# facebook/facebook360_dep

Measured on AMD Instinct MI355X. Metric: depth Mpix/s per GPU (full pyramid, 16-cam 2048^2 rig); % HBM-read roofline, higher is better.
Workload: dtype f32+f64; 1 GPU; BASELINE config 3: 16-camera 2048x2048 synthetic rig, 8-frame sequence, full 10-level pyramid per frame, per-level temporal filter (+-2 frames); the same sequence for every --gpus N (block partition, 8 frame(s) on this rank); rig=cfg2, cameras=16, frames=8, temporal_filter=True, halo_transport=local, parallelism=frames x1

## Files before the change

### facebook360_dep_amd/csrc/derp_capi.hip

```cpp
#include <hip/hip_runtime.h>

#include <algorithm>
#include <cfloat>
#include <cmath>
#include <cstdarg>
#include <cstdio>
#include <cstdlib>
#include <cstring>
#include <map>
#include <memory>
#include <string>
#include <vector>

#include <rocprim/device/device_radix_sort.hpp>

#include "../../include/derp_hip.h"
#include "derp_host.h"
#include "derp_kernels.h"
#include "derp_mesh.h"
#include "derp_points.h"
#include "derp_render.h"
#include "derp_geometric.h"
#include "derp_sweep.h"
#include "derp_align.h"
// ... 337 lines not shown
  return 0;
}

bool batch_needs_inverse_warps(const derp_ctx* c, int dst0, int nd) {
  std::vector<char> covered(c->S, 0);
  for (int d = dst0; d < dst0 + nd; ++d) {
    covered[c->dst2srcH[d]] = 1;
  }
  for (int s = 0; s < c->S; ++s) {
    if (!covered[s]) {
      return true;
    }
  }
  return false;
}

size_t table_bytes_per_dst(const derp_ctx* c, int W, int H, bool withInverse) {
  const size_t wp = (size_t)(W + 2 * kPadW) * (H + 2 * kPadW), cp = (size_t)(W + 2 * kPadC) * (H + 2 * kPadC);
  return (size_t)(c->S - 1) * (wp * sizeof(float2) + 2 * cp * sizeof(ushort4) + (withInverse ? (size_t)W * H * sizeof(float2) : 0) +
                               (DERP_RANDOM_TILED ? tiled_plane(W, H) * sizeof(ushort4) : 0));
}

int compute_fov_and_masks(derp_ctx* c, int level) {
  const int W = c->LW[level], H = c->LH[level];
  const size_t n = (size_t)W * H;
  {
    Span sp(c, ST_FOV, level);
    if (c->opt.rebuild_warp_tables || c->fovCachedLevel != level) {
      hipLaunchKernelGGL(k_fov_mask, grid2d(W, H, c->D, kBlk2d), kBlk2d, 0, c->stream, c->camsDst.as<Cam>(), W, H,
                         c->fovMask.as<uint8_t>());
      KCHECK(c);
      c->fovCachedLevel = level;
    }
    hipLaunchKernelGGL(k_and_masks, dim3(flat_grid(n), c->D), dim3(256), 0, c->stream, c->fovMask.as<uint8_t>(),
                       c->frame().fg[level].as<uint8_t>(), c->dst2src.as<int>(), 0, n, c->w.maskAnd.as<uint8_t>());
    KCHECK(c);
  }
  return 0;
}

int build_warp(derp_ctx* c, int dst0, int nd) {
  const int L = c->cur;
  Span sp(c, ST_PROJ_WARP, L);
  {
    const size_t n = (size_t)c->LW[L] * c->LH[L];
    ALLOC(c, c->rayDir, 3 * n * c->D * sizeof(double));
    ALLOC(c, c->behind, n * c->D * sizeof(unsigned));
  }
  LevelView V = make_view(c, ST_PROJ_WARP, dst0, nd);
  hipLaunchKernelGGL(k_proj_warp, grid2d(V.W + 2 * kPadW, V.H + 2 * kPadW, c->S, kBlk2d), kBlk2d, 0, c->stream, V,
                     c->projWarp.as<float2>());
  KCHECK(c);
  hipLaunchKernelGGL(k_pixel_rays, grid2d(V.W, V.H, nd, kBlk2d), kBlk2d, 0, c->stream, V, c->rayDir.as<double>(),
                     c->behind.as<unsigned>());
  KCHECK(c);
  c->w.colorTablesCleanLevel = -1;
  if (batch_needs_inverse_warps(c, dst0, nd)) {
    hipLaunchKernelGGL(k_proj_warp_inv, grid2d(V.W, V.H, nd, kBlk2d), kBlk2d, 0, c->stream, V, c->projWarpInv.as<float2>());
    KCHECK(c);
  }
  return 0;
}

int build_color_tables(derp_ctx* c, int dst0, int nd) {
  const int L = c->cur;
  LevelView V = make_view(c, ST_REPROJECT, dst0, nd);
  Span sp(c, ST_REPROJECT, L);
  const dim3 grid((V.W + kRbTile - 1) / kRbTile, (V.H + kRbTile - 1) / kRbTile, nd * (c->S - 1));
  ALLOC(c, c->w.tileSeen, (size_t)grid.x * grid.y * grid.z);
  const int skipBlank = c->w.colorTablesCleanLevel == L && nd == c->D && !c->noBlankSkip;
  const auto kernel = c->reprojectSerial ? k_reproject_bias : k_reproject_bias_front;
// ... 187 lines not shown
  return t * 4 * sizeof(float) + ((t + 3) & ~(size_t)3);
}

constexpr size_t kBilateralMaxLds = 64 * 1024 - 256;

bool bilateral_fast_tap_ok(float sigma, float w0, float w1, float w2) {
  const float denom = 2.0f * (sigma * sigma);
  return w1 == 1.0f && w2 == 1.0f && w0 >= 0.0f && std::isfinite(w0) && denom > 0.0f && std::isfinite(denom);
}

bool temporal_fast_tap_ok(float sigma, float w0, float w1, float w2) {
  const float sig2 = sigma * sigma;
  const auto weight_ok = [](float w) { return w >= 0.0f && std::isfinite(w); };
  return weight_ok(w0) && weight_ok(w1) && weight_ok(w2) && sig2 > 0.0f && std::isfinite(sig2);
}

void launch_joint_bilateral_u16_tiled(derp_ctx* c, dim3 grid, const float* image, const void* guide, const uint8_t* mask,
                                      int W, int H, int radius, float sigma, float w0, float w1, float w2, float* out,
                                      size_t planeStride, size_t guideStride, const int* guideIndex) {
  const bool fast = bilateral_fast_tap_ok(sigma, w0, w1, w2) && bilateral_lds_bytes(radius) + 256 <= kBilateralMaxLds;
  const auto kernel = fast ? k_joint_bilateral<true, true> : k_joint_bilateral<true, false>;
  hipLaunchKernelGGL(kernel, grid, dim3(256), bilateral_lds_bytes(radius), c->stream, image, guide, mask, W, H, radius, sigma,
                     w0, w1, w2, out, planeStride, guideStride, guideIndex);
}

int run_bilateral(derp_ctx* c) {
  const int L = c->cur;
  Span sp(c, ST_BILATERAL, L);
  c->randomRanThisLevel = false;
  const int W = c->LW[L], H = c->LH[L];
  const size_t n = (size_t)W * H;
  const int radius = bilateral_radius(L);
  launch_joint_bilateral_u16_tiled(c, dim3((W + 15) / 16, (H + 15) / 16, c->D), c->w.disparity.as<float>(),
                                   (const void*)c->frame().color[L].as<ushort4>(), c->w.maskAnd.as<uint8_t>(), W, H, radius,
                                   0.005f, 0.5f, 1.0f, 1.0f, c->w.tmpF.as<float>(), n, n, c->dst2src.as<int>());
  KCHECK(c);
  std::swap(c->w.disparity, c->w.tmpF);
  return 0;
}

int run_median(derp_ctx* c, bool fuseMaskFov, float* levelOut = nullptr) {
  const int L = c->cur;
  Span sp(c, ST_MEDIAN, L);
  c->randomRanThisLevel = false;
  const int W = c->LW[L], H = c->LH[L];
  const size_t n = (size_t)W * H;
  hipLaunchKernelGGL(k_masked_median, grid2d(W, H, c->D, kBlk2d), kBlk2d, 0, c->stream, c->w.disparity.as<float>(),
                     c->opt.use_foreground_masks ? c->frame().bg[L].as<float>() : (const float*)nullptr,
                     c->w.maskAnd.as<uint8_t>(), W, H, 1, levelOut ? levelOut : c->w.tmpF.as<float>(), n,
                     fuseMaskFov ? c->fovMask.as<uint8_t>() : (const uint8_t*)nullptr);
  KCHECK(c);
  if (!levelOut) {
    std::swap(c->w.disparity, c->w.tmpF);
  }
  return 0;
}

int run_mask_fov(derp_ctx* c, float* levelOut = nullptr) {
  const int L = c->cur;
  Span sp(c, ST_MASKFOV, L);
  const size_t n = npx(c, L) * c->D;
  hipLaunchKernelGGL(k_mask_fov, dim3(flat_grid(n)), dim3(256), 0, c->stream, c->w.disparity.as<float>(),
                     c->fovMask.as<uint8_t>(), levelOut ? levelOut : c->w.disparity.as<float>(), n);
  KCHECK(c);
  return 0;
}

int check_level(derp_ctx* c, int level) {
  if (!c || c->numLevels == 0) {
    return fail(c, "derp_set_pyramid has not been called");
  }
  if (level < 0 || level >= c->numLevels) {
    return fail(c, "level %d out of range [0, %d)", level, c->numLevels);
  }
  if (c->LW[level] <= 0 || c->LH[level] <= 0) {
    return fail(c, "level %d was declared absent in derp_set_pyramid", level);
  }
  return 0;
}

int level_begin(derp_ctx* c, int level, bool buildAllTables) {
  TRY(check_level(c, level));
// ... 253 lines not shown
  }
  if (n > kMaxTemporalFrames) {
    ALLOC(c, c->temporalCarry, (size_t)planes * W * H * sizeof(float2));
  }
  for (int t0 = 0; t0 < n; t0 += kMaxTemporalFrames) {
    TemporalFrames F;
    F.n = std::min(kMaxTemporalFrames, n - t0);
    for (int t = 0; t < F.n; ++t) {
      F.guides[t] = reinterpret_cast<const ushort4*>(guides[t0 + t]);
      F.images[t] = images[t0 + t];
      F.masks[t] = masks[t0 + t];
    }
    F.refGuide = reinterpret_cast<const ushort4*>(guides[centre]);
    F.refImage = images[centre];
    F.refMask = masks[centre];
    F.carry = n > kMaxTemporalFrames ? c->temporalCarry.as<float2>() : nullptr;
    F.first = t0 == 0;
    F.last = t0 + F.n >= n;
    const size_t lds = 2 * ((((size_t)(32 + 2 * radius) * (8 + 2 * radius) * 9) + 15) & ~(size_t)15);
    if (radius >= 0 && lds <= 48 * 1024 && !c->noTemporalTile) {
      const bool fast = temporal_fast_tap_ok(sigma, w0, w1, w2) && !c->temporalGeneric;
      const auto kernel = !fast ? k_temporal_tiled<-1, false> : radius == 1 ? k_temporal_tiled<1, true> : k_temporal_tiled<-1, true>;
      hipLaunchKernelGGL(kernel, grid2d(W, H, planes, kBlk2d), kBlk2d, lds, c->stream, F, W, H, sigma, radius, w0, w1, w2, out,
                         dst2src);
    } else {
      hipLaunchKernelGGL(k_temporal, grid2d(W, H, planes, kBlk2d), kBlk2d, 0, c->stream, F, W, H, sigma, radius, w0, w1, w2,
                         out, dst2src);
    }
    KCHECK(c);
  }
  return 0;
}

}

extern "C" {

void derp_options_default(derp_options* o) {
  o->min_depth_m = 0.5f;
  o->max_depth_m = 1e4f;
  o->var_noise_floor = 4e-5f;
  o->var_high_thresh = 1e-3f;
  o->random_proposals = 2;
  o->ping_pong_iterations = 1;
  o->mismatches_start_level = -1;
  o->do_bilateral_filter = 1;
  o->do_median_filter = 1;
  o->use_foreground_masks = 0;
  o->partial_coverage = 0;
  o->rebuild_warp_tables = 1;
}

int derp_create(derp_ctx** out, int device, const derp_camera_desc* src, int n_src, const derp_camera_desc* dst,
                int n_dst) {
  if (!out) {
    return 1;
  }
  *out = nullptr;
  std::unique_ptr<derp_ctx> owner(new derp_ctx);
  derp_ctx* c = owner.get();
  derp_options_default(&c->opt);
  if (n_src <= 0 || n_dst <= 0) {
    return create_fail("no source / destination cameras!");
  }
  hipDeviceProp_t prop;
  TRY(open_device(device, "the depth path", &prop));
  c->device = device;
  if (prop.maxSharedMemoryPerMultiProcessor > 0) {
    c->ldsPerCu = prop.maxSharedMemoryPerMultiProcessor;
  }
  if (const char* e = getenv("DERP_XCD_ROTATE")) {
    c->xcdRotate = atoi(e);
  }
  if (const char* e = getenv("DERP_XCD_BANDS")) {
    c->xcdBands = atoi(e);
  }
  if (const char* e = getenv("DERP_COST_TILES_PER_BLOCK")) {
    c->costTilesPerBlock = atoi(e);
  }
  c->noMemo = getenv("DERP_NO_MEMO") != nullptr;
  if (const char* e = getenv("DERP_BRUTE_RUN")) {
    c->bruteRun = atoi(e);
  }
  if (const char* e = getenv("DERP_PP_COMPACT")) {
    c->ppCompact = atoi(e) != 0;
  }
  if (const char* e = getenv("DERP_RANDOM_WAVES")) {
    c->randomWaves = atoi(e);
  }
  if (const char* e = getenv("DERP_PP_WAVES")) {
    c->ppWaves = atoi(e);
  }
  c->noTemporalTile = getenv("DERP_NO_TEMPORAL_TILE") != nullptr;
  c->noBlankSkip = getenv("DERP_NO_BLANK_SKIP") != nullptr;
  if (const char* e = getenv("DERP_TEMPORAL_GENERIC")) {
    c->temporalGeneric = atoi(e) != 0;
  }
  if (const char* e = getenv("DERP_REPROJECT_SERIAL")) {
    c->reprojectSerial = atoi(e) != 0;
  }
  c->S = n_src;
  c->D = n_dst;
  c->frames.resize(1);
  c->camsSrcH.resize(n_src);
  c->camsDstH.resize(n_dst);
  for (int i = 0; i < n_src; ++i) {
    if (const char* m = host_prepare_camera(src[i], c->camsSrcH[i])) {
      return create_fail(std::string("camera ") + src[i].id + ": " + m);
    }
  }
  c->dst2srcH.assign(n_dst, 0);
  c->descDstH.assign(dst, dst + n_dst);
  for (int i = 0; i < n_dst; ++i) {
    if (const char* m = host_prepare_camera(dst[i], c->camsDstH[i])) {
      return create_fail(std::string("camera ") + dst[i].id + ": " + m);
    }
    bool found = false;
    for (int s = 0; s < n_src; ++s) {
      if (strncmp(dst[i].id, src[s].id, sizeof dst[i].id) == 0) {
        c->dst2srcH[i] = s;
        found = true;
        break;
      }
    }
    if (!found) {
      return create_fail(std::string("destination camera ") + dst[i].id + " is not a source camera");
    }
    if (memcmp(&c->camsDstH[i], &c->camsSrcH[c->dst2srcH[i]], sizeof(Cam)) != 0) {
      return create_fail(std::string("destination camera ") + dst[i].id + " differs from the source camera of the same id "
                  "(destinations must be cameras of the source rig, as filterDestinations makes them)");
// ... 451 lines not shown
```

### facebook360_dep_amd/csrc/derp_ctx.h

```cpp
#pragma once

namespace {

enum Stage {
  ST_FOV = 0,
  ST_VARIANCE,
  ST_OWN_BIAS,
  ST_UPSAMPLE,
  ST_PROJ_WARP,
  ST_REPROJECT,
  ST_PROJ_BIAS,
  ST_BRUTE,
  ST_RANDOM,
  ST_PINGPONG,
  ST_MISMATCH,
  ST_BILATERAL,
  ST_MEDIAN,
  ST_MASKFOV,
  ST_TEMPORAL,
  ST_LANES,
  ST_GC_PREPARE,
  ST_GC_SWEEP,
  ST_GC_CLEAN,
  ST_SWEEP_OVERLAPS,
// ... 86 lines not shown
  DevBuf temporalCarry;
  DevBuf projWarp, projWarpInv;
  DevBuf rayDir, behind;
  int warpCachedLevel = -1;
  DevBuf fovMask;
  int fovCachedLevel = -1;
  bool randomRanThisLevel = false;
  bool tablesValid = false;
  std::map<std::pair<int, int>, LanczosTab> lanczos;
  std::map<std::pair<int, int>, AreaTabDev> areaTabs;
  DevBuf spiral;
  int spiralN = 0, spiralRadius = -1;
  std::vector<std::unique_ptr<WorkLane>> lanes;
  hipEvent_t laneReady = nullptr;
  int activeLane = -1;

  DevBuf counters;
  bool profiling = false;
  std::vector<TimedSpan> spans;
  double accMs[ST_COUNT][kMaxLevels] = {};
  int accLaunch[ST_COUNT][kMaxLevels] = {};
  int xcdRotate = 1;
  int xcdBands = 0, costTilesPerBlock = 0;
  DevBuf blockTrace[2][kMaxLevels];
  int blockTraceGrid[2][kMaxLevels][2] = {};
  bool noMemo = false;
  int bruteRun = 10;
  bool ppCompact = true;
  int randomWaves = 0, ppWaves = 0;
  size_t ldsPerCu = 160 * 1024;
  bool noTemporalTile = false;
  bool noBlankSkip = false;
  bool temporalGeneric = false, reprojectSerial = false;
  std::unique_ptr<SmrState> smr;
  std::unique_ptr<RephotoState> rephoto;
  std::unique_ptr<PointsState> points;
  std::unique_ptr<MeshState> mesh;
  std::unique_ptr<GcState> gc;
  std::unique_ptr<SweepState> sweep;
  std::unique_ptr<AlignState> align;
};

namespace {

int fail(derp_ctx* c, const char* fmt, ...) {
  va_list ap;
  va_start(ap, fmt);
  vfail(c ? &c->err : nullptr, fmt, ap);
  va_end(ap);
  return 1;
}

int use_device(derp_ctx* c) {
  if (!c) {
    return 1;
  }
  HIPCHK(c, hipSetDevice(c->device));
  return 0;
}

int check_camera(derp_ctx* c, int cam) {
  if (cam < 0 || cam >= c->D) {
    return fail(c, "bad camera index %d (the context has %d)", cam, c->D);
  }
  return 0;
}
// ... 3 lines not shown
```

### facebook360_dep_amd/csrc/derp_kernels.h

```cpp
#pragma once
#include <hip/hip_runtime.h>
#include <math.h>
#include <stdint.h>

#include <type_traits>

#include "derp_camera.h"
#include "gcc_algos.h"

namespace derp {

#ifndef DERP_COST_MIN_WAVES
#define DERP_COST_MIN_WAVES 4
#endif
#ifndef DERP_RANDOM_MIN_WAVES
#define DERP_RANDOM_MIN_WAVES 4
#endif
#ifndef DERP_RANDOM_TILED
#define DERP_RANDOM_TILED 0
#endif
#ifndef DERP_MIX_HOT_ONLY
#define DERP_MIX_HOT_ONLY 0
#endif
#ifndef DERP_PHASE_TIMERS
// ... 3013 lines not shown
        }
      } else {
        for (int u = -radius; u <= radius; ++u) {
          for (int v = -radius; v <= radius; ++v) {
            const int k = ((int)threadIdx.y + radius + v) * TW + (int)threadIdx.x + radius + u;
            if (!tm[k]) {
              continue;
            }
            temporal_tap<FAST>(ref, tg[k], centre, weight0, weight1, weight2, rcpSig2, expTab, weightedSumPix, sumWeight);
          }
        }
      }
    }
    if (t + 1 < F.n) {
      stash(t + 1);
    }
  }
  if (!inside) {
    return;
  }
  if (!active) {
    if (F.last) {
      out[pd + idx] = F.refImage[pd + idx];
    }
    return;
  }
  if (F.last) {
    out[pd + idx] = weightedSumPix / sumWeight;
  } else {
    F.carry[pd + idx] = make_float2(weightedSumPix, sumWeight);
  }
}

__global__ void k_rephoto_splat(const Cam* __restrict__ cams, int target, const float* __restrict__ disps, int W, int H,
                                unsigned long long* __restrict__ key) {
  const int x = blockIdx.x * blockDim.x + threadIdx.x, y = blockIdx.y * blockDim.y + threadIdx.y;
  const int j = blockIdx.z;
  if (x >= W || y >= H || j == target) {
    return;
  }
  const size_t n = (size_t)W * H, idx = (size_t)y * W + x;
  const float d = disps[(size_t)j * n + idx];
  if (!(d > 0) || isinf(d)) {
    return;
  }
  const Cam& cj = cams[j];
  const Cam& ct = cams[target];
  const D3 dir = rig_direction(cj, (x + 0.5) / (double)W, (y + 0.5) / (double)H, cj.principal[0], cj.principal[1],
                               cj.focal[0], cj.focal[1]);
  const double depth = (double)(1.0f / d);
  const D3 p = {cj.pos[0] + dir.x * depth, cj.pos[1] + dir.y * depth, cj.pos[2] + dir.z * depth};
  D2 pn;
  if (!sees(ct, p, ct.principal[0], ct.principal[1], ct.focal[0], ct.focal[1], 1.0, 1.0, pn)) {
    return;
  }
  const double px = pn.x * (double)W, py = pn.y * (double)H;
  const double dx = p.x - ct.pos[0], dy = p.y - ct.pos[1], dz = p.z - ct.pos[2];
  const float dist = (float)sqrt(sum3(dx * dx, dy * dy, dz * dz));
  const unsigned long long k =
      ((unsigned long long)__float_as_uint(dist) << 32) | ((unsigned long long)j << 24) | (unsigned long long)idx;
  const int x0 = (int)floor(px - 0.5), y0 = (int)floor(py - 0.5);
  for (int yy = y0; yy <= y0 + 1; ++yy) {
    for (int xx = x0; xx <= x0 + 1; ++xx) {
      if (xx >= 0 && yy >= 0 && xx < W && yy < H) {
        atomicMin(&key[(size_t)yy * W + xx], k);
      }
// ... 412 lines not shown
```

### facebook360_dep_amd/csrc/derp_sequence.h

```cpp
#pragma once
#include <dlfcn.h>
#include <rccl/rccl.h>

namespace {

void seq_window(int t, int first, int last, int radius, int* lo, int* hi) {
  *lo = std::max(first, t - radius);
  *hi = std::min(last, t + radius);
}

int seq_owner(int first, int last, int world, int policy, int frame) {
  const int F = last - first + 1, i = frame - first;
  if (i < 0 || i >= F || world < 1) {
    return -1;
  }
  if (policy == DERP_SEQ_CYCLIC) {
    return i % world;
  }
  const int q = F / world, r = F % world;
  const int big = r * (q + 1);
  return i < big ? i / (q + 1) : r + (q ? (i - big) / q : 0);
}

std::vector<derp_seq_transfer> seq_plan(int first, int last, int world, int radius, int policy) {
// ... 49 lines not shown
  auto sym = [&](const char* n) {
    void* p = dlsym(api.lib, n);
    if (!p && api.error.empty()) {
      api.error = std::string("librccl lacks ") + n;
    }
    return p;
  };
  api.GetUniqueId = reinterpret_cast<decltype(api.GetUniqueId)>(sym("ncclGetUniqueId"));
  api.CommInitRank = reinterpret_cast<decltype(api.CommInitRank)>(sym("ncclCommInitRank"));
  api.CommDestroy = reinterpret_cast<decltype(api.CommDestroy)>(sym("ncclCommDestroy"));
  api.GroupStart = reinterpret_cast<decltype(api.GroupStart)>(sym("ncclGroupStart"));
  api.GroupEnd = reinterpret_cast<decltype(api.GroupEnd)>(sym("ncclGroupEnd"));
  api.Send = reinterpret_cast<decltype(api.Send)>(sym("ncclSend"));
  api.Recv = reinterpret_cast<decltype(api.Recv)>(sym("ncclRecv"));
  api.GetErrorString = reinterpret_cast<decltype(api.GetErrorString)>(sym("ncclGetErrorString"));
  if (!api.error.empty()) {
    api.lib = nullptr;
  }
  return &api;
}

enum { SEQ_NONE = 0, SEQ_LOOPBACK = 1, SEQ_RCCL = 2, SEQ_EXTERNAL = 3 };

}

struct derp_seq {
  derp_ctx* c = nullptr;
  int first = 0, last = 0, rank = 0, world = 1;
  derp_seq_options opt;
  std::vector<int> owned, halo;
  std::vector<derp_seq_transfer> plan;
  std::vector<std::vector<DevBuf>> haloColor, haloFg, haloDisp;
  std::vector<DevBuf> filtered;
  DevBuf fov, winMask;
  int transport = SEQ_NONE;
  std::vector<derp_seq*> peers;
  ncclComm_t comm = nullptr;
  unsigned long long bytesSent = 0, bytesRecv = 0;
  std::vector<std::pair<hipEvent_t, hipEvent_t>> exchangeSpans;
  double exchangeMs = 0;
  hipStream_t xStream = nullptr;
  hipEvent_t computedEv = nullptr, exchangedEv = nullptr;
  bool exchangePending = false;
  std::vector<std::pair<hipEvent_t, hipEvent_t>> waitSpans;
  double exchangeExposedMs = 0;
  int levelReady = -1;
  int levelExchanged = -1;
  int computeLevel = -1, computedFrames = 0;
  std::vector<int> computedAt, filteredAt;
  std::vector<uint64_t> uploaded;
  std::vector<hipEvent_t> filteredEv;
  int fovLevel = -1;
  bool streaming = false;
  int nSlots = 0;
  struct HostIn {
    const uint16_t* color = nullptr;
    const uint8_t* fg = nullptr;
    const float* bg = nullptr;
  };
  std::vector<std::vector<HostIn>> hostIn;
  std::vector<std::vector<float*>> hostDisp;
  std::vector<char> hostHave;
  std::vector<float*> hostRaw;
  struct SlotTag {
    int k = -1, colorLevel = -1, rawLevel = -1;
  };
  std::vector<SlotTag> slotTag;
// ... 309 lines not shown
  if (hipSetDevice(c->device) != hipSuccess) {
    return fail(c, "hipSetDevice failed");
  }
  const int nOwned = (int)q->owned.size();
  q->streaming = q->opt.resident_frames > 0 && q->opt.resident_frames < nOwned;
  q->nSlots = q->streaming ? q->opt.resident_frames : std::max(1, nOwned);
  if (q->streaming && q->opt.do_temporal_filter && q->nSlots < 2 * q->opt.time_radius + 1) {
    return fail(c, "resident_frames %d is smaller than the temporal window (2 * time_radius + 1 = %d frames)",
                q->nSlots, 2 * q->opt.time_radius + 1);
  }
  TRY(derp_set_frame_slots(c, q->nSlots));
  const int nl = c->numLevels;
  for (auto* vv : {&q->haloColor, &q->haloFg, &q->haloDisp}) {
    vv->resize(q->halo.size());
    for (auto& v : *vv) {
      v.resize(nl);
    }
  }
  size_t nmax = 0;
  for (int l = 0; l < nl; ++l) {
    const size_t n = npx(c, l);
    nmax = std::max(nmax, n);
    if (n == 0) {
      continue;
    }
    for (size_t h = 0; h < q->halo.size(); ++h) {
      if (q->haloColor[h][l].ensure(n * c->S * sizeof(ushort4)) || q->haloDisp[h][l].ensure(n * c->D * sizeof(float)) ||
          (q->opt.use_foreground_masks && q->haloFg[h][l].ensure(n * c->S))) {
        return fail(c, "out of device memory allocating the temporal halo (frame %d, level %d)", q->halo[h], l);
      }
    }
  }
  q->filtered.resize(q->streaming ? 1 : q->owned.size());
  q->computedAt.assign(q->owned.size(), -1);
  q->filteredAt.assign(q->owned.size(), -1);
  if (hipStreamCreateWithFlags(&q->xStream, hipStreamNonBlocking) != hipSuccess ||
      hipEventCreateWithFlags(&q->computedEv, hipEventDisableTiming) != hipSuccess ||
      hipEventCreateWithFlags(&q->exchangedEv, hipEventDisableTiming) != hipSuccess) {
    return fail(c, "hipStreamCreate / hipEventCreate failed");
  }
  q->filteredEv.assign(q->streaming ? 0 : q->owned.size(), nullptr);
  for (auto& e : q->filteredEv) {
    if (hipEventCreateWithFlags(&e, hipEventDisableTiming) != hipSuccess) {
      return fail(c, "hipEventCreate failed");
    }
  }
  for (auto& b : q->filtered) {
    if (b.ensure(nmax * c->D * sizeof(float))) {
      return fail(c, "out of device memory allocating the filtered level");
    }
  }
  if (q->streaming) {
    q->slotTag.assign(q->nSlots, derp_seq::SlotTag());
    q->hostIn.assign(nOwned, std::vector<derp_seq::HostIn>(nl));
    q->hostDisp.assign(nOwned, std::vector<float*>(nl, nullptr));
    q->hostHave.assign((size_t)nOwned * nl, 0);
    q->hostRaw.assign(nOwned, nullptr);
    for (int k = 0; k < nOwned; ++k) {
      if (q->opt.do_temporal_filter && hipHostMalloc((void**)&q->hostRaw[k], nmax * c->D * sizeof(float), hipHostMallocDefault) != hipSuccess) {
        q->hostRaw[k] = nullptr;
        return fail(c, "out of page-locked host memory for the raw level of frame %d", q->owned[k]);
      }
      for (int l = 0; l < nl; ++l) {
        const size_t n = npx(c, l);
        if (n && hipHostMalloc((void**)&q->hostDisp[k][l], n * c->D * sizeof(float), hipHostMallocDefault) != hipSuccess) {
          q->hostDisp[k][l] = nullptr;
          return fail(c, "out of page-locked host memory for the results of frame %d", q->owned[k]);
        }
      }
    }
    for (const derp_seq_transfer& tr : q->plan) {
      if (tr.from_rank == rank && (q->edge.empty() || q->edge.back() != tr.frame)) {
        q->edge.push_back(tr.frame);
      }
    }
    for (auto* vv : {&q->edgeColor, &q->edgeFg}) {
      vv->resize(q->edge.size());
      for (auto& v : *vv) {
        v.resize(nl);
      }
    }
    q->edgeRaw.resize(q->edge.size());
    for (size_t e = 0; e < q->edge.size(); ++e) {
      if (q->edgeRaw[e].ensure(nmax * c->D * sizeof(float))) {
        return fail(c, "out of device memory allocating the edge frames");
      }
      for (int l = 0; l < nl; ++l) {
        const size_t n = npx(c, l);
        if (n && (q->edgeColor[e][l].ensure(n * c->S * sizeof(ushort4)) ||
                  (q->opt.use_foreground_masks && q->edgeFg[e][l].ensure(n * c->S)))) {
          return fail(c, "out of device memory allocating the edge frames");
        }
      }
    }
  }
  if (q->fov.ensure(nmax * c->D) ||
      (q->opt.use_foreground_masks && q->winMask.ensure((size_t)(2 * q->opt.time_radius + 1) * nmax * c->D))) {
    return fail(c, "out of device memory allocating the temporal masks");
  }
  *out = owner.release();
  return 0;
}

void derp_seq_destroy(derp_seq* q) {
  if (!q) {
    return;
  }
  if (q->c) {
    (void)hipSetDevice(q->c->device);
    (void)hipStreamSynchronize(q->c->stream);
  }
  seq_drain_spans(q);
  if (q->comm) {
    (void)rccl_api()->CommDestroy(q->comm);
  }
  for (auto& e : q->filteredEv) {
    if (e) {
      (void)hipEventDestroy(e);
    }
  }
  if (q->xStream) {
    (void)hipStreamSynchronize(q->xStream);
    (void)hipStreamDestroy(q->xStream);
  }
  for (hipEvent_t e : {q->computedEv, q->exchangedEv}) {
    if (e) {
      (void)hipEventDestroy(e);
    }
  }
  for (auto& v : q->hostDisp) {
// ... 629 lines not shown
  if (q->levelReady != level) {
    return fail(c, "derp_seq_level_exchange(%d): derp_seq_level_compute(%d) has not completed for every owned frame", level, level);
  }
  TRY(seq_exchange(q, level, 2));
  if (q->transport != SEQ_EXTERNAL) {
    q->levelExchanged = level;
  }
  if (q->streaming || getenv("DERP_SEQ_NO_OVERLAP")) {
    TRY(seq_join_exchange(q));
  }
  return 0;
}

int derp_seq_mark_exchanged(derp_seq* q, int level) {
  if (!q) {
    return 1;
  }
  q->levelExchanged = level;
  return 0;
}

namespace {
int seq_fov_masks(derp_seq* q, int level) {
  derp_ctx* c = q->c;
  if (q->fovLevel != level) {
    const int W = c->LW[level], H = c->LH[level];
    hipLaunchKernelGGL(k_fov_mask, grid2d(W, H, c->D, kBlk2d), kBlk2d, 0, c->stream, c->camsDst.as<Cam>(), W, H,
                       q->fov.as<uint8_t>());
    KCHECK(c);
    q->fovLevel = level;
  }
  return 0;
}
int seq_filter_frame(derp_seq* q, int level, int k) {
  derp_ctx* c = q->c;
  const int W = c->LW[level], H = c->LH[level];
  const size_t n = (size_t)W * H;
  const int radius = temporal_space_radius(q, level);
  const int t = q->owned[k];
  int lo, hi;
  seq_window(t, q->first, q->last, q->opt.time_radius, &lo, &hi);
  std::vector<const void*> wg(hi - lo + 1);
  std::vector<const float*> wi(hi - lo + 1);
  std::vector<const uint8_t*> wmk(hi - lo + 1);
  for (int u = lo; u <= hi; ++u) {
    void *pc, *pd, *pm;
    size_t b;
    TRY(seq_buffer(q, u, level, 0, &pc, &b));
    TRY(seq_buffer(q, u, level, 2, &pd, &b));
    if (q->opt.use_foreground_masks) {
      TRY(seq_buffer(q, u, level, 1, &pm, &b));
      uint8_t* wm = q->winMask.as<uint8_t>() + (size_t)(u - lo) * n * c->D;
      hipLaunchKernelGGL(k_and_masks, dim3(flat_grid(n), c->D), dim3(256), 0, c->stream, q->fov.as<uint8_t>(),
                         (const uint8_t*)pm, c->dst2src.as<int>(), 0, n, wm);
      KCHECK(c);
      pm = wm;
    } else {
      pm = q->fov.p;
    }
    wg[u - lo] = pc;
    wi[u - lo] = reinterpret_cast<const float*>(pd);
    wmk[u - lo] = reinterpret_cast<const uint8_t*>(pm);
  }
  TRY(temporal_launch(c, wg.data(), wi.data(), wmk.data(), hi - lo + 1, t - lo, W, H, c->D, q->opt.sigma, radius,
                      q->opt.weight_b, q->opt.weight_g, q->opt.weight_b, q->filtered[k].as<float>(), c->dst2src.as<int>()));
  q->filteredAt[k] = level;
  HIPCHK(c, hipEventRecord(q->filteredEv[k], c->stream));
  return 0;
}
}

int derp_seq_level_filter_frame(derp_seq* q, int level, int frame) {
  if (!q) {
    return 1;
  }
  derp_ctx* c = q->c;
  HIPCHK(c, hipSetDevice(c->device));
  TRY(check_level(c, level));
  const int k = owned_index(q, frame);
  if (k < 0) {
    return fail(c, "frame %d is not owned by rank %d", frame, q->rank);
  }
  if (!q->opt.do_temporal_filter || q->streaming) {
    return 2;
  }
  if (q->filteredAt[k] == level) {
    return 0;
  }
  int lo, hi;
  seq_window(frame, q->first, q->last, q->opt.time_radius, &lo, &hi);
  bool needsHalo = false;
  for (int u = lo; u <= hi; ++u) {
    const int ku = owned_index(q, u);
    if (ku >= 0 ? q->computedAt[ku] != level : q->levelExchanged != level) {
      return 2;
    }
    needsHalo |= ku < 0;
  }
  if (needsHalo) {
    TRY(seq_join_exchange(q));
  }
  Span sp(c, ST_TEMPORAL, level);
  TRY(seq_fov_masks(q, level));
  return seq_filter_frame(q, level, k);
}

int derp_seq_download_filtered(derp_seq* q, int frame, int level, int d, float* out) {
  if (!q) {
    return 1;
  }
  derp_ctx* c = q->c;
  TRY(check_level(c, level));
  const int k = owned_index(q, frame);
  if (k < 0 || d < -1 || d >= c->D || !out) {
    return fail(c, "bad frame / destination index / null output");
  }
  if (q->streaming || q->filteredAt[k] != level) {
    return fail(c, "frame %d has no filtered level %d in its scratch (derp_seq_level_filter_frame)", frame, level);
  }
  HIPCHK(c, hipSetDevice(c->device));
  const size_t n = npx(c, level);
  HIPCHK(c, hipStreamWaitEvent(c->copyStream, q->filteredEv[k], 0));
  HIPCHK(c, hipMemcpyAsync(out, q->filtered[k].as<float>() + (size_t)std::max(d, 0) * n, (d < 0 ? c->D : 1) * n * sizeof(float),
                           hipMemcpyDeviceToHost, c->copyStream));
  HIPCHK(c, hipStreamSynchronize(c->copyStream));
  return 0;
}

int derp_seq_level_filter(derp_seq* q, int level) {
  if (!q) {
    return 1;
  }
  derp_ctx* c = q->c;
  HIPCHK(c, hipSetDevice(c->device));
  TRY(check_level(c, level));
  if (!q->opt.do_temporal_filter) {
    return 0;
  }
  if (q->levelReady != level) {
    return fail(c, "derp_seq_level_filter(%d): derp_seq_level_compute(%d) has not completed for every owned frame", level, level);
  }
  if (!q->halo.empty() && q->levelExchanged != level) {
    return fail(c, "derp_seq_level_filter(%d): the halo frames' level has not been exchanged (derp_seq_level_exchange, or "
                   "derp_seq_mark_exchanged after an external transport moved it)", level);
  }
  const int W = c->LW[level], H = c->LH[level];
  const size_t n = (size_t)W * H;
  Span sp(c, ST_TEMPORAL, level);
  TRY(seq_fov_masks(q, level));
  if (q->streaming) {
    TRY(seq_join_exchange(q));
    const int radius = temporal_space_radius(q, level);
    TRY(stream_filter_level(q, level, W, H, radius));
    q->levelReady = -1;
    return 0;
  }
  for (int pass = 0; pass < 2; ++pass) {
    if (pass == 1) {
      TRY(seq_join_exchange(q));
    }
    for (int k = 0; k < (int)q->owned.size(); ++k) {
      if (q->filteredAt[k] == level) {
        continue;
      }
      int lo, hi;
      seq_window(q->owned[k], q->first, q->last, q->opt.time_radius, &lo, &hi);
      bool allOwned = true;
      for (int u = lo; allOwned && u <= hi; ++u) {
        allOwned = owned_index(q, u) >= 0;
      }
      if (pass == 1 || allOwned) {
        TRY(seq_filter_frame(q, level, k));
      }
    }
  }
  for (int k = 0; k < (int)q->owned.size(); ++k) {
    HIPCHK(c, hipMemcpyAsync(c->frames[k].disp[level].p, q->filtered[k].p, n * c->D * sizeof(float), hipMemcpyDeviceToDevice,
                             c->stream));
    q->computedAt[k] = -1;
  }
  q->levelReady = -1;
  return 0;
}

int derp_seq_run(derp_seq* q, int level_start, int level_end_) {
  if (!q) {
    return 1;
  }
  derp_ctx* c = q->c;
  if (level_start < level_end_) {
    return fail(c, "Check failed: level_start >= level_end (%d vs %d)", level_start, level_end_);
  }
  if (!q->plan.empty() && q->transport != SEQ_RCCL) {
    return fail(c, "derp_seq_run drives all three phases itself and needs the RCCL transport; with loopback / "
                   "external transports call derp_seq_level_compute / _exchange / _filter per level");
  }
  for (int level = level_start; level >= level_end_; --level) {
    TRY(derp_seq_level_compute(q, level));
    TRY(derp_seq_level_exchange(q, level));
    TRY(derp_seq_level_filter(q, level));
  }
  return 0;
}

int derp_seq_stats(derp_seq* q, uint64_t* bytes_sent, uint64_t* bytes_received, double* exchange_ms) {
  if (!q) {
    return 1;
  }
  HIPCHK(q->c, hipStreamSynchronize(q->c->stream));
  seq_drain_spans(q);
  if (bytes_sent) {
// ... 37 lines not shown
```

Before: 538.9 Mpix/s.

## Batch temporal filter across frames in one launch and write outputs in place

Adds a multi-frame temporal kernel that stages the union of window frames into LDS once per tile and produces several frames' outputs from it, replacing per-frame launches that reload overlapping neighbours. Outputs are written straight into the disparity buffers when nobody reads them later, removing the scratch buffer and device-to-device copy. It also skips the per-level AND-mask pass when foreground masks are off, using the FOV mask directly. This costs larger LDS footprint per block (possibly lower occupancy), more registers for the raw array, and more complex scheduling bookkeeping.

```diff
diff --git a/facebook360_dep_amd/csrc/derp_capi.hip b/facebook360_dep_amd/csrc/derp_capi.hip
--- a/facebook360_dep_amd/csrc/derp_capi.hip
+++ b/facebook360_dep_amd/csrc/derp_capi.hip
@@ -393,11 +393,17 @@
       KCHECK(c);
       c->fovCachedLevel = level;
     }
-    hipLaunchKernelGGL(k_and_masks, dim3(flat_grid(n), c->D), dim3(256), 0, c->stream, c->fovMask.as<uint8_t>(),
-                       c->frame().fg[level].as<uint8_t>(), c->dst2src.as<int>(), 0, n, c->w.maskAnd.as<uint8_t>());
-    KCHECK(c);
-  }
-  return 0;
+    if (c->opt.use_foreground_masks || c->levelMaskPass) {
+      hipLaunchKernelGGL(k_and_masks, dim3(flat_grid(n), c->D), dim3(256), 0, c->stream, c->fovMask.as<uint8_t>(),
+                         c->frame().fg[level].as<uint8_t>(), c->dst2src.as<int>(), 0, n, c->w.maskAnd.as<uint8_t>());
+      KCHECK(c);
+    }
+  }
+  return 0;
+}
+
+const uint8_t* level_mask(derp_ctx* c) {
+  return c->opt.use_foreground_masks || c->levelMaskPass ? c->w.maskAnd.as<uint8_t>() : c->fovMask.as<uint8_t>();
 }
 
 int build_warp(derp_ctx* c, int dst0, int nd) {
@@ -651,7 +657,7 @@
   const size_t n = (size_t)W * H;
   const int radius = bilateral_radius(L);
   launch_joint_bilateral_u16_tiled(c, dim3((W + 15) / 16, (H + 15) / 16, c->D), c->w.disparity.as<float>(),
-                                   (const void*)c->frame().color[L].as<ushort4>(), c->w.maskAnd.as<uint8_t>(), W, H, radius,
+                                   (const void*)c->frame().color[L].as<ushort4>(), level_mask(c), W, H, radius,
                                    0.005f, 0.5f, 1.0f, 1.0f, c->w.tmpF.as<float>(), n, n, c->dst2src.as<int>());
   KCHECK(c);
   std::swap(c->w.disparity, c->w.tmpF);
@@ -666,7 +672,7 @@
   const size_t n = (size_t)W * H;
   hipLaunchKernelGGL(k_masked_median, grid2d(W, H, c->D, kBlk2d), kBlk2d, 0, c->stream, c->w.disparity.as<float>(),
                      c->opt.use_foreground_masks ? c->frame().bg[L].as<float>() : (const float*)nullptr,
-                     c->w.maskAnd.as<uint8_t>(), W, H, 1, levelOut ? levelOut : c->w.tmpF.as<float>(), n,
+                     level_mask(c), W, H, 1, levelOut ? levelOut : c->w.tmpF.as<float>(), n,
                      fuseMaskFov ? c->fovMask.as<uint8_t>() : (const uint8_t*)nullptr);
   KCHECK(c);
   if (!levelOut) {
@@ -986,6 +992,46 @@
   return 0;
 }
 
+int temporal_frames_max_union(const derp_ctx* c, int radius) {
+  if (radius < 0 || c->noTemporalTile || c->temporalPerFrame) {
+    return 0;
+  }
+  const size_t buf = (((size_t)(32 + 2 * radius) * (8 + 2 * radius) * 9) + 15) & ~(size_t)15;
+  const size_t budget = std::min((size_t)c->ldsPerCu / 4, (size_t)48 * 1024) - 512;
+  return (int)std::min((size_t)kMaxTemporalUnion, budget / buf);
+}
+
+int temporal_frames_launch(derp_ctx* c, const void* const* guides, const float* const* images, const uint8_t* const* masks,
+                           int n, const int* self, const int* lo, const int* hi, float* const* out, int nOut, int W, int H,
+                           int planes, float sigma, int radius, float w0, float w1, float w2, const int* dst2src) {
+  if (n < 1 || n > temporal_frames_max_union(c, radius) || nOut < 1 || nOut > kMaxTemporalUnion) {
+    return fail(c, "temporal chunk of %d outputs over %d window frames does not fit one launch (radius %d)", nOut, n, radius);
+  }
+  TemporalChunk C;
+  for (int t = 0; t < n; ++t) {
+    C.guides[t] = reinterpret_cast<const ushort4*>(guides[t]);
+    C.images[t] = images[t];
+    C.masks[t] = masks[t];
+  }
+  for (int o = 0; o < nOut; ++o) {
+    if (lo[o] < 0 || hi[o] >= n || self[o] < lo[o] || self[o] > hi[o] || !out[o]) {
+      return fail(c, "temporal chunk: output %d has a window outside the staged frames", o);
+    }
+    C.self[o] = self[o];
+    C.lo[o] = lo[o];
+    C.hi[o] = hi[o];
+    C.out[o] = out[o];
+  }
+  C.nFrames = n;
+  C.nOut = nOut;
+  const size_t lds = (size_t)n * ((((size_t)(32 + 2 * radius) * (8 + 2 * radius) * 9) + 15) & ~(size_t)15);
+  const bool fast = temporal_fast_tap_ok(sigma, w0, w1, w2) && !c->temporalGeneric;
+  const auto kernel = !fast ? k_temporal_frames<-1, false> : radius == 1 ? k_temporal_frames<1, true> : k_temporal_frames<-1, true>;
+  hipLaunchKernelGGL(kernel, grid2d(W, H, planes, kBlk2d), kBlk2d, lds, c->stream, C, W, H, sigma, radius, w0, w1, w2, dst2src);
+  KCHECK(c);
+  return 0;
+}
+
 }
 
 extern "C" {
@@ -1050,6 +1096,15 @@
   if (const char* e = getenv("DERP_TEMPORAL_GENERIC")) {
     c->temporalGeneric = atoi(e) != 0;
   }
+  if (const char* e = getenv("DERP_TEMPORAL_PER_FRAME")) {
+    c->temporalPerFrame = atoi(e) != 0;
+  }
+  if (const char* e = getenv("DERP_LEVEL_MASK_PASS")) {
+    c->levelMaskPass = atoi(e) != 0;
+  }
+  if (const char* e = getenv("DERP_TEMPORAL_CHUNK")) {
+    c->temporalChunk = std::min(std::max(atoi(e), 1), kMaxTemporalUnion);
+  }
   if (const char* e = getenv("DERP_REPROJECT_SERIAL")) {
     c->reprojectSerial = atoi(e) != 0;
   }
diff --git a/facebook360_dep_amd/csrc/derp_ctx.h b/facebook360_dep_amd/csrc/derp_ctx.h
--- a/facebook360_dep_amd/csrc/derp_ctx.h
+++ b/facebook360_dep_amd/csrc/derp_ctx.h
@@ -142,6 +142,9 @@
   bool noTemporalTile = false;
   bool noBlankSkip = false;
   bool temporalGeneric = false, reprojectSerial = false;
+  bool temporalPerFrame = false;
+  int temporalChunk = 8;
+  bool levelMaskPass = false;
   std::unique_ptr<SmrState> smr;
   std::unique_ptr<RephotoState> rephoto;
   std::unique_ptr<PointsState> points;
diff --git a/facebook360_dep_amd/csrc/derp_kernels.h b/facebook360_dep_amd/csrc/derp_kernels.h
--- a/facebook360_dep_amd/csrc/derp_kernels.h
+++ b/facebook360_dep_amd/csrc/derp_kernels.h
@@ -3069,6 +3069,171 @@
   }
 }
 
+constexpr int kMaxTemporalUnion = 12;
+struct TemporalChunk {
+  const ushort4* guides[kMaxTemporalUnion];
+  const float* images[kMaxTemporalUnion];
+  const uint8_t* masks[kMaxTemporalUnion];
+  float* out[kMaxTemporalUnion];
+  int self[kMaxTemporalUnion], lo[kMaxTemporalUnion], hi[kMaxTemporalUnion];
+  int nFrames, nOut;
+};
+template <int RADIUS, bool FAST>
+__global__ void __launch_bounds__(256)
+    k_temporal_frames(TemporalChunk C, int W, int H, float sigma, int radiusArg, float weight0, float weight1,
+                      float weight2, const int* __restrict__ dst2src) {
+  extern __shared__ unsigned char ldsTemporal[];
+  __shared__ unsigned long long expTab[32];
+  __shared__ unsigned notFullBits;
+  const int tid = threadIdx.y * blockDim.x + threadIdx.x;
+  if (tid < 32) {
+    expTab[tid] = kExp2fTab[tid];
+  }
+  if (tid == 0) {
+    notFullBits = 0;
+  }
+  const int radius = RADIUS >= 0 ? RADIUS : radiusArg;
+  const int TW = 32 + 2 * radius, TH = 8 + 2 * radius, cells = TW * TH;
+  const size_t bufBytes = ((size_t)cells * 9 + 15) & ~(size_t)15;
+  const int x0 = blockIdx.x * 32, y0 = blockIdx.y * 8;
+  const int x = x0 + threadIdx.x, y = y0 + threadIdx.y;
+  const bool inside = x < W && y < H;
+  const size_t n = (size_t)W * H;
+  const size_t pd = (size_t)blockIdx.z * n, pg = dst2src ? (size_t)dst2src[blockIdx.z] * n : 0;
+  const size_t idx = inside ? (size_t)y * W + x : 0;
+  int cellSrc[2];
+#pragma unroll
+  for (int i = 0; i < 2; ++i) {
+    const int k = min(tid + i * 256, cells - 1);
+    const int ty = k / TW, tx = k - ty * TW;
+    const int sx = min(max(x0 - radius + tx, 0), W - 1), sy = min(max(y0 - radius + ty, 0), H - 1);
+    cellSrc[i] = sy * W + sx;
+  }
+  __syncthreads();
+  float raw[kMaxTemporalUnion];
+  unsigned myNotFull = 0;
+#pragma unroll
+  for (int g = 0; g < kMaxTemporalUnion; g += 4) {
+    if (g < C.nFrames) {
+      ushort4 sg[4][2];
+      unsigned char sm[4][2];
+#pragma unroll
+      for (int j = 0; j < 4; ++j) {
+        const int f = min(g + j, C.nFrames - 1);
+        const uint8_t* __restrict__ mask = C.masks[f] + pd;
+        const ushort4* __restrict__ guide = C.guides[f] + pg;
+#pragma unroll
+        for (int i = 0; i < 2; ++i) {
+          sm[j][i] = mask[cellSrc[i]];
+          sg[j][i] = guide[cellSrc[i]];
+        }
+        raw[g + j] = C.images[f][pd + idx];
+      }
+#pragma unroll
+      for (int j = 0; j < 4; ++j) {
+        const int f = g + j;
+        if (f < C.nFrames) {
+          unsigned char* buf = ldsTemporal + (size_t)f * bufBytes;
+          ushort4* tg = reinterpret_cast<ushort4*>(buf);
+          unsigned char* tm = buf + (size_t)cells * 8;
+          bool full = true;
+#pragma unroll
+          for (int i = 0; i < 2; ++i) {
+            const int k = tid + i * 256;
+            if (k < cells) {
+              full &= sm[j][i] != 0;
+              tm[k] = sm[j][i];
+              tg[k] = sg[j][i];
+            }
+          }
+          if (cells > 512) {
+            const uint8_t* __restrict__ mask = C.masks[f] + pd;
+            const ushort4* __restrict__ guide = C.guides[f] + pg;
+            for (int k = tid + 512; k < cells; k += 256) {
+              const int ty = k / TW, tx = k - ty * TW;
+              const int sx = min(max(x0 - radius + tx, 0), W - 1), sy = min(max(y0 - radius + ty, 0), H - 1);
+              const size_t j2 = (size_t)sy * W + sx;
+              const unsigned char mk = mask[j2];
+              full &= mk != 0;
+              tm[k] = mk;
+              tg[k] = guide[j2];
+            }
+          }
+          myNotFull |= full ? 0u : 1u << f;
+        }
+      }
+    }
+  }
+  if (FAST && myNotFull) {
+    atomicOr(&notFullBits, myNotFull);
+  }
+  __syncthreads();
+  if (!inside) {
+    return;
+  }
+  const unsigned notFull = FAST ? notFullBits : ~0u;
+  const float sig2 = sigma * sigma;
+  const double rcpSig2 = 1.0 / (double)sig2;
+  const int own = ((int)threadIdx.y + radius) * TW + (int)threadIdx.x + radius;
+  for (int o = 0; o < C.nOut; ++o) {
+    const int T = C.self[o];
+    float* out = C.out[o];
+    const unsigned char* bufT = ldsTemporal + (size_t)T * bufBytes;
+    if (!(bufT + (size_t)cells * 8)[own]) {
+      float v = raw[0];
+#pragma unroll
+      for (int j = 1; j < kMaxTemporalUnion; ++j) {
+        v = T == j ? raw[j] : v;
+      }
+      out[pd + idx] = v;
+      continue;
+    }
+    const ushort4 ref = reinterpret_cast<const ushort4*>(bufT)[own];
+    float weightedSumPix = 0.f, sumWeight = 0.f;
+    for (int f = C.lo[o]; f <= C.hi[o]; ++f) {
+      const unsigned char* buf = ldsTemporal + (size_t)f * bufBytes;
+      const ushort4* tg = reinterpret_cast<const ushort4*>(buf);
+      const unsigned char* tm = buf + (size_t)cells * 8;
+      float centre = raw[0];
+#pragma unroll
+      for (int j = 1; j < kMaxTemporalUnion; ++j) {
+        centre = f == j ? raw[j] : centre;
+      }
+      if (FAST && !((notFull >> f) & 1u)) {
+        if (RADIUS == 1) {
+          const ushort4* tc = tg + own;
+#pragma unroll
+          for (int u = -1; u <= 1; ++u) {
+#pragma unroll
+            for (int v = -1; v <= 1; ++v) {
+              temporal_tap<true>(ref, tc[v * (32 + 2) + u], centre, weight0, weight1, weight2, rcpSig2, expTab,
+                                 weightedSumPix, sumWeight);
+            }
+          }
+        } else {
+          for (int u = -radius; u <= radius; ++u) {
+            for (int v = -radius; v <= radius; ++v) {
+              temporal_tap<true>(ref, tg[own + v * TW + u], centre, weight0, weight1, weight2, rcpSig2, expTab,
+                                 weightedSumPix, sumWeight);
+            }
+          }
+        }
+      } else {
+        for (int u = -radius; u <= radius; ++u) {
+          for (int v = -radius; v <= radius; ++v) {
+            const int k = own + v * TW + u;
+            if (!tm[k]) {
+              continue;
+            }
+            temporal_tap<FAST>(ref, tg[k], centre, weight0, weight1, weight2, rcpSig2, expTab, weightedSumPix, sumWeight);
+          }
+        }
+      }
+    }
+    out[pd + idx] = weightedSumPix / sumWeight;
+  }
+}
+
 __global__ void k_rephoto_splat(const Cam* __restrict__ cams, int target, const float* __restrict__ disps, int W, int H,
                                 unsigned long long* __restrict__ key) {
   const int x = blockIdx.x * blockDim.x + threadIdx.x, y = blockIdx.y * blockDim.y + threadIdx.y;
diff --git a/facebook360_dep_amd/csrc/derp_sequence.h b/facebook360_dep_amd/csrc/derp_sequence.h
--- a/facebook360_dep_amd/csrc/derp_sequence.h
+++ b/facebook360_dep_amd/csrc/derp_sequence.h
@@ -105,7 +105,10 @@
   std::vector<derp_seq_transfer> plan;
   std::vector<std::vector<DevBuf>> haloColor, haloFg, haloDisp;
   std::vector<DevBuf> filtered;
+  std::vector<char> inPlace;
+  size_t scratchBytes = 0;
   DevBuf fov, winMask;
+  std::vector<int> maskAt;
   int transport = SEQ_NONE;
   std::vector<derp_seq*> peers;
   ncclComm_t comm = nullptr;
@@ -481,6 +484,9 @@
     }
   }
   q->filtered.resize(q->streaming ? 1 : q->owned.size());
+  q->inPlace.assign(q->owned.size(), 0);
+  q->maskAt.assign(q->owned.size() + q->halo.size(), -1);
+  q->scratchBytes = nmax * c->D * sizeof(float);
   q->computedAt.assign(q->owned.size(), -1);
   q->filteredAt.assign(q->owned.size(), -1);
   if (hipStreamCreateWithFlags(&q->xStream, hipStreamNonBlocking) != hipSuccess ||
@@ -494,10 +500,8 @@
       return fail(c, "hipEventCreate failed");
     }
   }
-  for (auto& b : q->filtered) {
-    if (b.ensure(nmax * c->D * sizeof(float))) {
-      return fail(c, "out of device memory allocating the filtered level");
-    }
+  if (q->streaming && q->filtered[0].ensure(q->scratchBytes)) {
+    return fail(c, "out of device memory allocating the filtered level");
   }
   if (q->streaming) {
     q->slotTag.assign(q->nSlots, derp_seq::SlotTag());
@@ -544,7 +548,8 @@
     }
   }
   if (q->fov.ensure(nmax * c->D) ||
-      (q->opt.use_foreground_masks && q->winMask.ensure((size_t)(2 * q->opt.time_radius + 1) * nmax * c->D))) {
+      (q->opt.use_foreground_masks &&
+       q->winMask.ensure(std::max((size_t)(2 * q->opt.time_radius + 1), q->streaming ? 0 : q->owned.size() + q->halo.size()) * nmax * c->D))) {
     return fail(c, "out of device memory allocating the temporal masks");
   }
   *out = owner.release();
@@ -1240,8 +1245,15 @@
   }
   return 0;
 }
+int seq_scratch(derp_seq* q, int k) {
+  if (q->filtered[k].ensure(q->scratchBytes)) {
+    return fail(q->c, "out of device memory allocating the filtered level of frame %d", q->owned[k]);
+  }
+  return 0;
+}
 int seq_filter_frame(derp_seq* q, int level, int k) {
   derp_ctx* c = q->c;
+  TRY(seq_scratch(q, k));
   const int W = c->LW[level], H = c->LH[level];
   const size_t n = (size_t)W * H;
   const int radius = temporal_space_radius(q, level);
@@ -1270,10 +1282,168 @@
     wi[u - lo] = reinterpret_cast<const float*>(pd);
     wmk[u - lo] = reinterpret_cast<const uint8_t*>(pm);
   }
+  std::fill(q->maskAt.begin(), q->maskAt.end(), -1);
   TRY(temporal_launch(c, wg.data(), wi.data(), wmk.data(), hi - lo + 1, t - lo, W, H, c->D, q->opt.sigma, radius,
                       q->opt.weight_b, q->opt.weight_g, q->opt.weight_b, q->filtered[k].as<float>(), c->dst2src.as<int>()));
   q->filteredAt[k] = level;
+  q->inPlace[k] = 0;
   HIPCHK(c, hipEventRecord(q->filteredEv[k], c->stream));
+  return 0;
+}
+
+int seq_frame_mask(derp_seq* q, int level, int u, const uint8_t** mask) {
+  derp_ctx* c = q->c;
+  if (!q->opt.use_foreground_masks) {
+    *mask = q->fov.as<uint8_t>();
+    return 0;
+  }
+  const int ku = owned_index(q, u);
+  const int slot = ku >= 0 ? ku : (int)q->owned.size() + halo_index(q, u);
+  const size_t n = npx(c, level);
+  uint8_t* wm = q->winMask.as<uint8_t>() + (size_t)slot * n * c->D;
+  if (q->maskAt[slot] != level) {
+    void* pm;
+    size_t b;
+    TRY(seq_buffer(q, u, level, 1, &pm, &b));
+    hipLaunchKernelGGL(k_and_masks, dim3(flat_grid(n), c->D), dim3(256), 0, c->stream, q->fov.as<uint8_t>(),
+                       (const uint8_t*)pm, c->dst2src.as<int>(), 0, n, wm);
+    KCHECK(c);
+    q->maskAt[slot] = level;
+  }
+  *mask = wm;
+  return 0;
+}
+
+struct SeqFilterLaunch {
+  std::vector<int> outs;
+  std::vector<int> frames;
+  bool afterJoin = false;
+  bool perFrame = false;
+};
+
+int seq_filter_level(derp_seq* q, int level) {
+  derp_ctx* c = q->c;
+  const int W = c->LW[level], H = c->LH[level];
+  const int radius = temporal_space_radius(q, level);
+  const int maxUnion = temporal_frames_max_union(c, radius);
+  std::vector<SeqFilterLaunch> plan;
+  for (int pass = 0; pass < 2; ++pass) {
+    SeqFilterLaunch cur;
+    auto close = [&]() {
+      if (!cur.outs.empty()) {
+        cur.afterJoin = pass == 1;
+        plan.push_back(cur);
+      }
+      cur = SeqFilterLaunch();
+    };
+    for (int k = 0; k < (int)q->owned.size(); ++k) {
+      if (q->filteredAt[k] == level) {
+        continue;
+      }
+      int lo, hi;
+      seq_window(q->owned[k], q->first, q->last, q->opt.time_radius, &lo, &hi);
+      bool allOwned = true;
+      for (int u = lo; allOwned && u <= hi; ++u) {
+        allOwned = owned_index(q, u) >= 0;
+      }
+      if (allOwned != (pass == 0)) {
+        continue;
+      }
+      if (hi - lo + 1 > maxUnion) {
+        close();
+        cur.outs.push_back(k);
+        for (int u = lo; u <= hi; ++u) {
+          cur.frames.push_back(u);
+        }
+        cur.perFrame = true;
+        close();
+        continue;
+      }
+      std::vector<int> grown = cur.frames;
+      for (int u = lo; u <= hi; ++u) {
+        if (grown.empty() || grown.back() < u) {
+          grown.push_back(u);
+        }
+      }
+      if ((int)cur.outs.size() >= c->temporalChunk || (int)grown.size() > maxUnion) {
+        close();
+        grown.clear();
+        for (int u = lo; u <= hi; ++u) {
+          grown.push_back(u);
+        }
+      }
+      cur.outs.push_back(k);
+      cur.frames = grown;
+    }
+    close();
+  }
+  std::vector<char> sent(q->owned.size(), 0);
+  for (const derp_seq_transfer& tr : q->plan) {
+    const int k = tr.from_rank == q->rank ? owned_index(q, tr.frame) : -1;
+    if (k >= 0) {
+      sent[k] = 1;
+    }
+  }
+  bool joined = false;
+  for (size_t i = 0; i < plan.size(); ++i) {
+    const SeqFilterLaunch& L = plan[i];
+    if (L.afterJoin && !joined) {
+      TRY(seq_join_exchange(q));
+      joined = true;
+    }
+    if (L.perFrame) {
+      TRY(seq_filter_frame(q, level, L.outs[0]));
+      continue;
+    }
+    const int nf = (int)L.frames.size(), no = (int)L.outs.size();
+    std::vector<const void*> wg(nf);
+    std::vector<const float*> wi(nf);
+    std::vector<const uint8_t*> wmk(nf);
+    for (int f = 0; f < nf; ++f) {
+      void *pc, *pd;
+      size_t b;
+      TRY(seq_buffer(q, L.frames[f], level, 0, &pc, &b));
+      TRY(seq_buffer(q, L.frames[f], level, 2, &pd, &b));
+      TRY(seq_frame_mask(q, level, L.frames[f], &wmk[f]));
+      wg[f] = pc;
+      wi[f] = reinterpret_cast<const float*>(pd);
+    }
+    std::vector<int> self(no), wlo(no), whi(no);
+    std::vector<float*> out(no);
+    for (int o = 0; o < no; ++o) {
+      const int k = L.outs[o], t = q->owned[k];
+      int lo, hi;
+      seq_window(t, q->first, q->last, q->opt.time_radius, &lo, &hi);
+      const auto at = [&](int u) { return (int)(std::lower_bound(L.frames.begin(), L.frames.end(), u) - L.frames.begin()); };
+      self[o] = at(t);
+      wlo[o] = at(lo);
+      whi[o] = at(hi);
+      bool readLater = !joined && sent[k];
+      for (size_t j = i + 1; !readLater && j < plan.size(); ++j) {
+        readLater = std::binary_search(plan[j].frames.begin(), plan[j].frames.end(), t);
+      }
+      if (readLater) {
+        TRY(seq_scratch(q, k));
+        out[o] = q->filtered[k].as<float>();
+      } else {
+        out[o] = c->frames[k].disp[level].as<float>();
+      }
+      q->inPlace[k] = !readLater;
+    }
+    TRY(temporal_frames_launch(c, wg.data(), wi.data(), wmk.data(), nf, self.data(), wlo.data(), whi.data(), out.data(), no, W, H,
+                               c->D, q->opt.sigma, radius, q->opt.weight_b, q->opt.weight_g, q->opt.weight_b,
+                               c->dst2src.as<int>()));
+    for (int k : L.outs) {
+      q->filteredAt[k] = level;
+      if (q->inPlace[k]) {
+        q->computedAt[k] = -1;
+      }
+      HIPCHK(c, hipEventRecord(q->filteredEv[k], c->stream));
+    }
+  }
+  if (!joined) {
+    TRY(seq_join_exchange(q));
+  }
   return 0;
 }
 }
@@ -1329,7 +1499,8 @@
   HIPCHK(c, hipSetDevice(c->device));
   const size_t n = npx(c, level);
   HIPCHK(c, hipStreamWaitEvent(c->copyStream, q->filteredEv[k], 0));
-  HIPCHK(c, hipMemcpyAsync(out, q->filtered[k].as<float>() + (size_t)std::max(d, 0) * n, (d < 0 ? c->D : 1) * n * sizeof(float),
+  const float* held = q->inPlace[k] ? c->frames[k].disp[level].as<float>() : q->filtered[k].as<float>();
+  HIPCHK(c, hipMemcpyAsync(out, held + (size_t)std::max(d, 0) * n, (d < 0 ? c->D : 1) * n * sizeof(float),
                            hipMemcpyDeviceToHost, c->copyStream));
   HIPCHK(c, hipStreamSynchronize(c->copyStream));
   return 0;
@@ -1363,28 +1534,13 @@
     q->levelReady = -1;
     return 0;
   }
-  for (int pass = 0; pass < 2; ++pass) {
-    if (pass == 1) {
-      TRY(seq_join_exchange(q));
-    }
-    for (int k = 0; k < (int)q->owned.size(); ++k) {
-      if (q->filteredAt[k] == level) {
-        continue;
-      }
-      int lo, hi;
-      seq_window(q->owned[k], q->first, q->last, q->opt.time_radius, &lo, &hi);
-      bool allOwned = true;
-      for (int u = lo; allOwned && u <= hi; ++u) {
-        allOwned = owned_index(q, u) >= 0;
-      }
-      if (pass == 1 || allOwned) {
-        TRY(seq_filter_frame(q, level, k));
-      }
-    }
-  }
+  std::fill(q->maskAt.begin(), q->maskAt.end(), -1);
+  TRY(seq_filter_level(q, level));
   for (int k = 0; k < (int)q->owned.size(); ++k) {
-    HIPCHK(c, hipMemcpyAsync(c->frames[k].disp[level].p, q->filtered[k].p, n * c->D * sizeof(float), hipMemcpyDeviceToDevice,
-                             c->stream));
+    if (!q->inPlace[k]) {
+      HIPCHK(c, hipMemcpyAsync(c->frames[k].disp[level].p, q->filtered[k].p, n * c->D * sizeof(float), hipMemcpyDeviceToDevice,
+                               c->stream));
+    }
     q->computedAt[k] = -1;
   }
   q->levelReady = -1;
```

Result: no change. 543.2 Mpix/s, median of 6 (+0.8%).
